# tskare/gpuaudiobench

Hardware: AMD Instinct MI355X
Metric: audio_buffers_per_sec (higher is better)
Workload: dtype f32

## Files before the change

gpuaudiobench_amd/csrc/k_conv_accel.hip:

```cpp
#include <hip/hip_runtime.h>
#include <hip/hip_ext.h>

#include <cmath>
#include <cstdlib>
#include <algorithm>
#include <chrono>
#include <memory>
#include <mutex>
#include <string>
#include <thread>
#include <type_traits>
#include <utility>
#include <vector>

#include "gab_common.hpp"
#include "gab_fft.hpp"
#include "gab_plan.hpp"
#include "k_conv_fdl.hpp"

namespace gab {
namespace fft {

void build_twiddles(float* t) {
    for (int m = 0; m < kTwiddleN; ++m) {
// ... 385 lines not shown
__global__ __launch_bounds__(kThreads) void conv_split_carry_refresh_kernel(
    const float* __restrict__ hist, const float4* __restrict__ pmF, cf* __restrict__ carry,
    const cf* __restrict__ tw, int head) {
    __shared__ cf lds[2 * kLdsHalf];
    const int tid = threadIdx.x;
    const int q = blockIdx.x;
    const cf* const hp = reinterpret_cast<const cf*>(hist) + (size_t)q * kSlots * kB;
    cf* const cp = carry + (size_t)q * kCarrySlots * kB;
    using FB = fft::BlockFFT<kNB, 16, false>;
    using FBi = fft::BlockFFT<kNB, 16, true>;
    cf* const X = lds;
    cf* const Y = lds + kLdsHalf;
    cf zb[16];
    typename FB::Bases twb_base;
    FB::load_twiddles(twb_base, tw, tid);
#pragma unroll
    for (int r = 0; r < 16; ++r)
        zb[r] = hp[((head + 1 + (r >> 1)) & (kSlots - 1)) * kB + (r & 1) * kThreads + tid];
    float4 cb[16];
    load_spectra<kNB, 16>(cb, pmF + (size_t)q * kBinsB, tid);
    typename FB::Twiddles twb;
    FB::expand_twiddles(twb_base, twb);
    FB::run(zb, X, Y, twb, tid);
    cf zpb[16];
    partner_exchange<kNB, 16, true>(zb, zpb, X, tid);
    spectral_product<kNB, 16>(zb, zpb, cb, tid);
    FBi::template run<typename FB::Twiddles, 4>(zb, Y, X, twb, tid);
    cf* const c1 = cp + ((head + 1) & (kCarrySlots - 1)) * kB;
    cf* const c2 = cp + ((head + 2) & (kCarrySlots - 1)) * kB;
    c1[tid] = zb[12];
    c1[tid + kThreads] = zb[13];
    c2[tid] = zb[14];
    c2[tid + kThreads] = zb[15];
}

constexpr unsigned kRtSentinel = 0xffa5c3e1u;
__device__ __forceinline__ bool rt_pending(unsigned w) { return (w >> 24) == (kRtSentinel >> 24); }
constexpr size_t kRtUploadPiece = (size_t(4) << 20) - 256;
constexpr int kRtPollLimit = 1 << 21;
constexpr int kRtMaxGroups = 40;
constexpr size_t kBatchChunk = 256;
struct ConvRoundTrip {
    unsigned* stage;
    float* park;
    float* h_out;
    unsigned* counters;
    unsigned* done;
    const unsigned* landed;
    unsigned* error;
    unsigned epoch;
    int groups;
    unsigned bound[kRtMaxGroups + 1];
};

#ifdef GAB_ABLATE
__device__ unsigned long long g_rt_stamps[65 * 4];
#define GAB_RT_STAMP_MIN(g, i) do { if (threadIdx.x == 0) atomicMin(&g_rt_stamps[(g) * 4 + (i)], (unsigned long long)__builtin_amdgcn_s_memrealtime()); } while (0)
#define GAB_RT_STAMP_MAX(g, i) do { if (threadIdx.x == 0) atomicMax(&g_rt_stamps[(g) * 4 + (i)], (unsigned long long)__builtin_amdgcn_s_memrealtime()); } while (0)
#else
#define GAB_RT_STAMP_MIN(g, i) do {} while (0)
#define GAB_RT_STAMP_MAX(g, i) do {} while (0)
#endif

__device__ __forceinline__ unsigned rt_peek(const unsigned* p) {
    return __hip_atomic_load(p, __ATOMIC_RELAXED, __HIP_MEMORY_SCOPE_SYSTEM);
}
constexpr unsigned kRtErrWait = 1u, kRtErrTorn = 2u;

__global__ __launch_bounds__(kThreads) void conv_round_trip_check_kernel(unsigned* __restrict__ stage, const float* __restrict__ hist,
                                                                        unsigned* __restrict__ verdict, int slot) {
    const int tid = threadIdx.x, q = blockIdx.x;
    const cf* const hp = reinterpret_cast<const cf*>(hist) + ((size_t)q * kSlots + slot) * kB;
    unsigned* const row = stage + (size_t)(2 * q) * kB;
    const cf c0 = hp[tid], c1 = hp[tid + kThreads];
    const unsigned v0 = rt_peek(row + tid), v1 = rt_peek(row + tid + kThreads), v2 = rt_peek(row + kB + tid), v3 = rt_peek(row + kB + tid + kThreads);
    const bool torn = v0 != __float_as_uint(c0.x) || v2 != __float_as_uint(c0.y) || v1 != __float_as_uint(c1.x) || v3 != __float_as_uint(c1.y);
    if (torn) __hip_atomic_fetch_or(verdict, kRtErrTorn, __ATOMIC_RELAXED, __HIP_MEMORY_SCOPE_SYSTEM);
    __hip_atomic_store(row + tid, kRtSentinel, __ATOMIC_RELAXED, __HIP_MEMORY_SCOPE_SYSTEM);
    __hip_atomic_store(row + tid + kThreads, kRtSentinel, __ATOMIC_RELAXED, __HIP_MEMORY_SCOPE_SYSTEM);
    __hip_atomic_store(row + kB + tid, kRtSentinel, __ATOMIC_RELAXED, __HIP_MEMORY_SCOPE_SYSTEM);
    __hip_atomic_store(row + kB + tid + kThreads, kRtSentinel, __ATOMIC_RELAXED, __HIP_MEMORY_SCOPE_SYSTEM);
}

__global__ __launch_bounds__(kThreads, 2) void conv_round_trip_kernel(
    ConvRoundTrip rt, float* __restrict__ hist, const float4* __restrict__ pmA, const float4* __restrict__ pmB,
    const cf* __restrict__ tw, int T, int head) {
    __shared__ cf lds[2 * kLdsHalf];
    __shared__ int s_word;
    cf* const lds0 = lds;
    cf* const lds1 = lds + kLdsHalf;
    const int tid = threadIdx.x;
    const int q = blockIdx.x;
    const int ta = 2 * q;
    int g = 0;
    while (q >= (int)rt.bound[g + 1]) ++g;
    GAB_RT_STAMP_MIN(g, 0);
    cf* const hp = reinterpret_cast<cf*>(hist) + (size_t)q * kSlots * kB;
    using FA = fft::BlockFFT<kNA, 4, false>;
    using FAi = fft::BlockFFT<kNA, 4, true>;
    using FB = fft::BlockFFT<kNB, 16, false>;
    using FBi = fft::BlockFFT<kNB, 16, true>;

    cf zb[16];
    typename FB::Bases twb_base;
    FB::load_twiddles(twb_base, tw, tid);
#pragma unroll
    for (int r = 0; r < 16; ++r) zb[r] = hp[((head + (r >> 1)) & (kSlots - 1)) * kB + (r & 1) * kThreads + tid];
    const cf prev0 = zb[14], prev1 = zb[15];
    {
        float4 cb[16];
        load_spectra<kNB, 16>(cb, pmB + (size_t)q * kBinsB, tid);
        __builtin_amdgcn_sched_barrier(0);
        typename FB::Twiddles twb;
        FB::expand_twiddles(twb_base, twb);
        FB::run(zb, lds1, lds0, twb, tid);
        cf zpb[16];
        partner_exchange<kNB, 16, true>(zb, zpb, lds1, tid);
        spectral_product<kNB, 16>(zb, zpb, cb, tid);
        FBi::template run<typename FB::Twiddles, 2>(zb, lds0, lds1, twb, tid);
    }
    const cf far0 = zb[14], far1 = zb[15];

    float4 ca[4];
    load_spectra<kNA, 4>(ca, pmA + (size_t)q * kBinsA, tid);
    typename FA::Twiddles twa;
    {
        typename FA::Bases twa_base;
        FA::load_twiddles(twa_base, tw, tid);
        FA::expand_twiddles(twa_base, twa);
    }

    const unsigned* const row = rt.stage + (size_t)ta * kB;
    if (tid == 0) {
        int tries = 0, bad = 0;
        while (rt_pending(rt_peek(row + 2 * kB - 1))) {
            if ((++tries & 63) == 0 && rt_peek(rt.landed) == rt.epoch) break;
            if (tries > kRtPollLimit) { bad = 1; break; }
            __builtin_amdgcn_s_sleep(30);
        }
        s_word = bad;
    }
    __syncthreads();
    bool gave_up = s_word != 0;
    unsigned w[4];
    {
        int tries = 0;
        for (;;) {
            w[0] = rt_peek(row + tid);
            w[1] = rt_peek(row + tid + kThreads);
            w[2] = rt_peek(row + kB + tid);
            w[3] = rt_peek(row + kB + tid + kThreads);
            if (gave_up || !(rt_pending(w[0]) || rt_pending(w[1]) || rt_pending(w[2]) || rt_pending(w[3]))) break;
            if ((++tries & 15) == 0 && __hip_atomic_load(rt.landed, __ATOMIC_ACQUIRE, __HIP_MEMORY_SCOPE_SYSTEM) == rt.epoch) {
                w[0] = rt_peek(row + tid);
                w[1] = rt_peek(row + tid + kThreads);
                w[2] = rt_peek(row + kB + tid);
                w[3] = rt_peek(row + kB + tid + kThreads);
                break;
            }
            if (tries > kRtPollLimit) { gave_up = true; break; }
            __builtin_amdgcn_s_sleep(10);
        }
    }
    GAB_RT_STAMP_MAX(g, 1);
    if (gave_up) __hip_atomic_store(rt.error, kRtErrWait, __ATOMIC_RELAXED, __HIP_MEMORY_SCOPE_SYSTEM);

    cf za[4];
    za[0] = prev0;
    za[1] = prev1;
    za[2] = mk(__uint_as_float(w[0]), __uint_as_float(w[2]));
    za[3] = mk(__uint_as_float(w[1]), __uint_as_float(w[3]));
    hp[head * kB + tid] = za[2];
    hp[head * kB + kThreads + tid] = za[3];
    __syncthreads();
    FA::run(za, lds0, lds1, twa, tid);
    {
        cf zpa[4];
        partner_exchange<kNA, 4, true>(za, zpa, lds0, tid);
        spectral_product<kNA, 4>(za, zpa, ca, tid);
    }
    FAi::run(za, lds1, lds0, twa, tid);
    float ya0 = 0.f, yb0 = 0.f, ya1 = 0.f, yb1 = 0.f;
    ya0 += za[2].x; yb0 += za[2].y; ya1 += za[3].x; yb1 += za[3].y;
    ya0 += far0.x; yb0 += far0.y; ya1 += far1.x; yb1 += far1.y;

    {
        unsigned long long* const p0 = reinterpret_cast<unsigned long long*>(rt.park + (size_t)T * tid + ta);
        unsigned long long* const p1 = reinterpret_cast<unsigned long long*>(rt.park + (size_t)T * (tid + kThreads) + ta);
        const unsigned long long v0 = ((unsigned long long)__float_as_uint(yb0) << 32) | __float_as_uint(ya0);
        const unsigned long long v1 = ((unsigned long long)__float_as_uint(yb1) << 32) | __float_as_uint(ya1);
        __hip_atomic_store(p0, v0, __ATOMIC_RELAXED, __HIP_MEMORY_SCOPE_AGENT);
        __hip_atomic_store(p1, v1, __ATOMIC_RELAXED, __HIP_MEMORY_SCOPE_AGENT);
    }
    asm volatile("s_waitcnt vmcnt(0)" ::: "memory");
    __syncthreads();
    GAB_RT_STAMP_MAX(g, 2);
    const int first = rt.bound[g];
    const int members = (int)rt.bound[g + 1] - first;
    unsigned* const gw = rt.counters + 32 * g;
    if (tid == 0) {
        const unsigned old = __hip_atomic_fetch_add(&gw[0], 1u, __ATOMIC_RELAXED, __HIP_MEMORY_SCOPE_AGENT);
        int role = 1;
        if (old + 1u == rt.epoch * (unsigned)members) {
            role = 2;
            __hip_atomic_store(&gw[1], 0u, __ATOMIC_RELAXED, __HIP_MEMORY_SCOPE_AGENT);
            asm volatile("s_waitcnt vmcnt(0)" ::: "memory");
            __hip_atomic_store(&gw[2], rt.epoch, __ATOMIC_RELAXED, __HIP_MEMORY_SCOPE_AGENT);
        } else {
            int tries = 0;
            while (__hip_atomic_load(&gw[2], __ATOMIC_RELAXED, __HIP_MEMORY_SCOPE_AGENT) != rt.epoch) {
                if (++tries > (1 << 10)) { role = 0; break; }
                __builtin_amdgcn_s_sleep(3);
            }
        }
        s_word = role;
    }
    __syncthreads();
    const int role = s_word;
    if (role == 0) return;
    const int row_f4 = members / 2;
    const auto srd = __builtin_amdgcn_make_buffer_rsrc(rt.park, 0, (int)((size_t)T * kB * 4), 0x00020000);
    const int col0 = 2 * first;
    unsigned drained = 0;
    for (;;) {
        __syncthreads();
        if (tid == 0) s_word = (int)__hip_atomic_fetch_add(&gw[1], 1u, __ATOMIC_RELAXED, __HIP_MEMORY_SCOPE_AGENT);
        __syncthreads();
        const int share = s_word;
        if (share >= members) break;
        const int i = share * kThreads + tid;
        const int sidx = i / row_f4, c = i - sidx * row_f4;
        const auto raw = __builtin_amdgcn_raw_buffer_load_b128(srd, 4u * (unsigned)(T * sidx + col0 + 4 * c), 0, 16);
        typedef float f4v __attribute__((ext_vector_type(4)));
        const f4v val = {__uint_as_float(raw[0]), __uint_as_float(raw[1]), __uint_as_float(raw[2]), __uint_as_float(raw[3])};
        float* const dst = rt.h_out + (size_t)T * sidx + col0 + 4 * c;
        asm volatile("global_store_dwordx4 %0, %1, off sc0 sc1" ::"v"(dst), "v"(val) : "memory");
        ++drained;
        if (role != 2) break;
    }
    asm volatile("s_waitcnt vmcnt(0)" ::: "memory");
    __syncthreads();
    GAB_RT_STAMP_MAX(g, 3);
    if (tid == 0 && drained) {
        const unsigned old = __hip_atomic_fetch_add(&rt.counters[32 * rt.groups], drained, __ATOMIC_RELAXED, __HIP_MEMORY_SCOPE_AGENT);
        if (old + drained == rt.epoch * (unsigned)gridDim.x) {
            __hip_atomic_store(rt.done, rt.epoch, __ATOMIC_RELAXED, __HIP_MEMORY_SCOPE_SYSTEM);
            GAB_RT_STAMP_MAX(64, 0);
        }
    }
}

__global__ __launch_bounds__(kThreads, 2) void conv_batch_kernel(
    const float* __restrict__ in, float* __restrict__ out, float* __restrict__ hist,
    const float4* __restrict__ pmA, const float4* __restrict__ pmB,
    const cf* __restrict__ tw, int T, int head, int n_buffers) {
    __shared__ cf lds[2 * kLdsHalf];
    const size_t step = (size_t)T * kB;
    for (int nb = 0; nb < n_buffers; ++nb)
        conv_one_buffer<true, true, true>(in + nb * step, out + nb * step, hist, pmA, pmB, tw, T,
                                             (head + nb) & (kSlots - 1), lds);
}

constexpr int kBatchBarriers = 6;

struct ConvEngine {
    const unsigned* doorbell;
    unsigned* relay;
    unsigned* progress;
    unsigned* completed;
    unsigned* error;
    int ring;
    int poll_every_period;
    unsigned* started;
    unsigned* resident;
    unsigned long long idle_ticks;
};
constexpr double kEngineIdleSeconds = 4.0;

typedef unsigned u4 __attribute__((ext_vector_type(4)));

constexpr int kB12Threads = 768;
constexpr int kB12SpecCf = 4 * kBinsA * 2;
constexpr int kB12Tw1Cf = 16 * 15;
constexpr int kB12Lds = 6 * kWaveImg + 2 * kLdsHalf + kB12SpecCf + kB12Tw1Cf;

template <int N, int R, int R0, int R1, class PM>
__device__ __forceinline__ void load_spectra_part(float4 (&c)[R1 - R0], PM pm, int tid) {
    constexpr int NT = N / R;
#pragma unroll
    for (int r = R0; r < R1; ++r) {
        const int k = tid + r * NT;
        if (r < R / 2) c[r - R0] = pm[k];
        else if (r > R / 2) c[r - R0] = pm[N - k];
        else c[r - R0] = pm[tid == 0 ? k : N - k];
    }
}
template <int N, int R, int R0, int R1>
__device__ __forceinline__ void spectral_product_part(cf (&z)[R], const cf (&zraw)[R1 - R0], const float4 (&c)[R1 - R0], int tid) {
#pragma unroll
    for (int r = R0; r < R1; ++r) {
        cf P = mk(c[r - R0].x, c[r - R0].y), M = mk(c[r - R0].z, c[r - R0].w);
        if (r > R / 2 || (r == R / 2 && tid != 0)) z[r] = fft::cfma_cjcj(zraw[r - R0], M, fft::cmulc(z[r], P));
        else z[r] = fft::cfma_cj(zraw[r - R0], M, fft::cmul(z[r], P));
    }
}
template <int R0, int R1>
__device__ __forceinline__ void near_product_half(cf (&v)[16], const cf* fimg, const float4* sp_lds, int lane) {
    cf zp[R1 - R0];
    float4 ch[R1 - R0];
#pragma unroll
    for (int r = R0; r < R1; ++r) zp[r - R0] = fimg[PadA16::at((kNA - (lane + 64 * r)) & (kNA - 1))];
    load_spectra_part<kNA, 16, R0, R1>(ch, sp_lds, lane);
    spectral_product_part<kNA, 16, R0, R1>(v, zp, ch, lane);
}

#ifdef GAB_ABLATE
__device__ unsigned long long g_split_stamps[2 * 8 * 8192];
#define GAB_B12BAR(period, i)                                                                                         \
    do {                                                                                                              \
        if ((sp.debug & 64) && ((period) == 32 || (period) == 33) && lane == 0)                                       \
            g_split_stamps[(((size_t)blockIdx.x * 12 + w) * 2 + ((period) - 32)) * 6 + (i)] = __builtin_amdgcn_s_memrealtime(); \
        __syncthreads();                                                                                              \
    } while (0)
#else
#define GAB_B12BAR(period, i) __syncthreads()
#endif
__device__ __forceinline__ void conv_split_batch12_resident(
    const float* __restrict__ in, float* __restrict__ out, float* __restrict__ hist,
    const float4* __restrict__ pmA, const ConvSplit& sp, const cf* __restrict__ tw, int T, int head0, int n_buffers,
    cf* __restrict__ lds) {
    cf* const far_img = lds + 6 * kWaveImg;
    float4* const spec = reinterpret_cast<float4*>(far_img + 2 * kLdsHalf);
    cf* const tw1 = reinterpret_cast<cf*>(spec + 4 * kBinsA);
    const int tid = threadIdx.x;
    const int d = xcd_contiguous(blockIdx.x, gridDim.x);
    const size_t step = (size_t)T * kB;
    {
        const float4* const gA = pmA + (size_t)(2 * d) * kBinsA;
        const float4* const gA2 = sp.pmA2 + (size_t)(2 * d) * kBinsA;
        for (int i = tid; i < 2 * kBinsA; i += kB12Threads) { spec[i] = gA[i]; spec[2 * kBinsA + i] = gA2[i]; }
        if (tid < 16) {
            cf pw[15];
            fft::powers_of<16>(tw[tid * (fft::kTwiddleN / 256)], pw);
#pragma unroll
            for (int r = 0; r < 15; ++r) tw1[tid * 15 + r] = pw[r];
        }
    }
    __syncthreads();
    const int lane = tid & 63;
    const int w = __builtin_amdgcn_readfirstlane(tid >> 6);
    const unsigned rb = (unsigned)lane + ((unsigned)lane >> 4);
    auto in_slot = [&](int slot) -> const float* { return in + (size_t)slot * step; };
    auto idle_period = [&]() { for (int i = 0; i < kBatchBarriers; ++i) __syncthreads(); };

    if (w >= 4) {
        const int g = __builtin_amdgcn_readfirstlane((w - 4) >> 2);
        const int ft = (tid - kThreads) & (kThreads - 1);
        cf* const img = far_img + g * kLdsHalf;
        const int q = 2 * d + g;
        const cf* const hp = reinterpret_cast<const cf*>(hist) + (size_t)q * kSlots * kB;
        cf* const cg = sp.carry + (size_t)q * kCarrySlots * kB;
        const size_t ca = (size_t)(2 * q) * kB, cb_ = ca + kB;
        const float4* const pf = sp.pmF + (size_t)q * kBinsB;
        using B16 = fft::Butterfly<16, false>;
        using B16i = fft::Butterfly<16, true>;
        cf tw2[15];
        fft::powers_of<16>(tw[ft], tw2);
        auto opaque_t = [&]() -> unsigned { unsigned v = (unsigned)ft; asm volatile("" : "+v"(v)); return v; };
        auto w0_of = [](unsigned t) -> unsigned { return t * 17u; };
        auto rd_of = [](unsigned t) -> unsigned { return t + (t >> 4); };
        auto w1_of = [](unsigned t) -> unsigned { const unsigned b1 = (t >> 4) * 256u + (t & 15u); return b1 + (b1 >> 4); };
        auto tw1row_of = [&](unsigned t) -> const cf* { return tw1 + (t & 15u) * 15u; };
        auto load_window = [&](auto part_tag, int nb, cf (&z)[16]) {
            constexpr int PART = decltype(part_tag)::value;
            const int head = (head0 + nb) & (kSlots - 1);
            int fo = ft;
            asm volatile("" : "+v"(fo));
            if constexpr (PART == 0) {
                const float* const cur = in_slot(nb);
                z[14] = mk(cur[ca + fo], cur[cb_ + fo]);
                z[15] = mk(cur[ca + fo + kThreads], cur[cb_ + fo + kThreads]);
            }
            constexpr int BL0 = PART == 0 ? 4 : 0, BL1 = PART == 0 ? 7 : 4;
            if (nb >= kSlots - 1) {
#pragma unroll
                for (int bl = BL0; bl < BL1; ++bl) {
                    const float* const src = in_slot(nb - (7 - bl));
                    z[2 * bl] = mk(src[ca + fo], src[cb_ + fo]);
                    z[2 * bl + 1] = mk(src[ca + fo + kThreads], src[cb_ + fo + kThreads]);
                }
            } else {
#pragma unroll
                for (int bl = BL0; bl < BL1; ++bl) {
                    if (nb - 7 + bl >= 0) {
                        const float* const src = in_slot(nb - (7 - bl));
                        z[2 * bl] = mk(src[ca + fo], src[cb_ + fo]);
                        z[2 * bl + 1] = mk(src[ca + fo + kThreads], src[cb_ + fo + kThreads]);
                    } else {
                        const int s = ((head + 1 + bl) & (kSlots - 1)) * kB;
                        z[2 * bl] = hp[s + fo];
                        z[2 * bl + 1] = hp[s + kThreads + fo];
                    }
                }
            }
        };
        cf z[16], zn[16];
        auto first_half = [&](int nb) {
#pragma unroll
            for (int r = 0; r < 16; ++r) z[r] = zn[r];
            B16::run(z);
            {
                const unsigned w0 = w0_of(opaque_t());
#pragma unroll
                for (int r = 0; r < 16; ++r) img[w0 + r] = z[B16::out_slot(r)];
            }
            GAB_B12BAR(nb, 0);
            {
                const unsigned t = opaque_t(), rd = rd_of(t);
                const cf* const tw1row = tw1row_of(t);
#pragma unroll
                for (int r = 0; r < 16; ++r) z[r] = img[rd + 272 * r];
#pragma unroll
                for (int r = 1; r < 16; ++r) z[r] = fft::cmul(z[r], tw1row[r - 1]);
            }
            B16::run(z);
            GAB_B12BAR(nb, 1);
            {
                const unsigned w1 = w1_of(opaque_t());
#pragma unroll
                for (int r = 0; r < 16; ++r) img[w1 + 17 * r] = z[B16::out_slot(r)];
            }
            __builtin_amdgcn_sched_barrier(0);
            float4 clo[8], chi[8];
            {
                int fo = ft;
                asm volatile("" : "+v"(fo));
                load_spectra_part<kNB, 16, 0, 8>(clo, pf, fo);
            }
            __builtin_amdgcn_sched_barrier(0);
            GAB_B12BAR(nb, 2);
            {
                const unsigned rd = rd_of(opaque_t());
#pragma unroll
                for (int r = 0; r < 16; ++r) z[r] = img[rd + 272 * r];
            }
#pragma unroll
            for (int r = 1; r < 16; ++r) z[r] = fft::cmul(z[r], tw2[r - 1]);
            __builtin_amdgcn_sched_barrier(0);
            {
                int fo = ft;
                asm volatile("" : "+v"(fo));
                load_spectra_part<kNB, 16, 8, 16>(chi, pf, fo);
            }
            __builtin_amdgcn_sched_barrier(0);
            B16::run(z);
            GAB_B12BAR(nb, 3);
            {
                const unsigned t = opaque_t();
#pragma unroll
                for (int r = 0; r < 16; ++r) img[t + 256u * r] = z[B16::out_slot(r)];
            }
            GAB_B12BAR(nb, 4);
            {
                cf o[16];
#pragma unroll
                for (int r = 0; r < 16; ++r) o[r] = z[B16::out_slot(r)];
#pragma unroll
                for (int r = 0; r < 16; ++r) z[r] = o[r];
                const unsigned t = opaque_t();
                const cf* const pb = img + (kNB - 256 * 15) - t;
                cf zp[8];
                zp[0] = img[(kNB - t) & (kNB - 1)];
#pragma unroll
                for (int r = 1; r < 8; ++r) zp[r] = pb[256 * (15 - r)];
                spectral_product_part<kNB, 16, 0, 8>(z, zp, clo, ft);
#pragma unroll
                for (int r = 0; r < 8; ++r) zp[r] = pb[256 * (7 - r)];
                spectral_product_part<kNB, 16, 8, 16>(z, zp, chi, ft);
            }
            B16i::run(z);
            GAB_B12BAR(nb, 5);
        };
        auto second_half = [&](int period, int nb_done, int nb_next) {
            if (nb_next >= 0) {
                load_window(std::integral_constant<int, 0>{}, nb_next, zn);
            } else {
#pragma unroll
                for (int r = 0; r < 16; ++r) zn[r] = mk(0.0f, 0.0f);
            }
            GAB_B12BAR(period, 0);
            if (nb_done >= 0) {
                const unsigned w0 = w0_of(opaque_t());
#pragma unroll
                for (int r = 0; r < 16; ++r) img[w0 + r] = z[B16i::out_slot(r)];
            }
            GAB_B12BAR(period, 1);
            if (nb_done >= 0) {
                const unsigned t = opaque_t(), rd = rd_of(t);
                const cf* const tw1row = tw1row_of(t);
#pragma unroll
                for (int r = 0; r < 16; ++r) z[r] = img[rd + 272 * r];
#pragma unroll
                for (int r = 1; r < 16; ++r) z[r] = fft::cmulc(z[r], tw1row[r - 1]);
                B16i::run(z);
            }
            GAB_B12BAR(period, 2);
            if (nb_done >= 0) {
                const unsigned w1 = w1_of(opaque_t());
#pragma unroll
                for (int r = 0; r < 16; ++r) img[w1 + 17 * r] = z[B16i::out_slot(r)];
            }
            __builtin_amdgcn_sched_barrier(0);
            if (nb_next >= 0) load_window(std::integral_constant<int, 1>{}, nb_next, zn);
            __builtin_amdgcn_sched_barrier(0);
            GAB_B12BAR(period, 3);
            if (nb_done >= 0) {
                const unsigned rd = rd_of(opaque_t());
#pragma unroll
                for (int r = 0; r < 16; ++r) z[r] = img[rd + 272 * r];
#pragma unroll
                for (int r = 1; r < 16; ++r) z[r] = fft::cmulc(z[r], tw2[r - 1]);
                cf x12, x13, x14, x15;
                B16i::run_last4(z, x12, x13, x14, x15);
                const int head = (head0 + nb_done) & (kSlots - 1);
                cf* const c1 = cg + ((head + 1) & (kCarrySlots - 1)) * kB;
                cf* const c2 = cg + ((head + 2) & (kCarrySlots - 1)) * kB;
                c1[ft] = x12;
                c1[ft + kThreads] = x13;
                c2[ft] = x14;
                c2[ft + kThreads] = x15;
            }
            GAB_B12BAR(period, 4);
            if (nb_done >= 0) asm volatile("s_waitcnt vmcnt(0)" ::: "memory");
            GAB_B12BAR(period, 5);
        };
        const int first = (g - head0) & 1;
        int nb = 0;
        if (first == 0 && n_buffers > 0) {
            load_window(std::integral_constant<int, 0>{}, 0, zn);
            load_window(std::integral_constant<int, 1>{}, 0, zn);
        }
        __syncthreads();
        if (first == 1) {
            second_half(0, -1, 1 < n_buffers ? 1 : -1);
            nb = 1;
        }
        for (;;) {
            if (nb > n_buffers) break;
            if (nb < n_buffers) first_half(nb); else idle_period();
            ++nb;
            if (nb > n_buffers) break;
            second_half(nb, nb - 1 < n_buffers ? nb - 1 : -1, nb + 1 < n_buffers ? nb + 1 : -1);
            ++nb;
        }
    } else if (w < 2) {
        const int q = 2 * d + w;
        cf* const hp = reinterpret_cast<cf*>(hist) + (size_t)q * kSlots * kB;
        cf* const img = lds + w * kWaveImg;
        cf* const hand = lds + (2 + w) * kWaveImg;
        const float4* const sa = spec + w * kBinsA;
        const float4* const sa2 = spec + (2 + w) * kBinsA;
        using WF = fft::WaveFFT1024<false>;
        WF::Lean t;
        WF::load_twiddles(t, tw, lane);
        const size_t xoff = (size_t)(2 * q) * kB;
        cf z[16], prev[8], nxt[8];
        {
            const int s1 = ((head0 + kSlots - 1) & (kSlots - 1)) * kB, s2 = ((head0 + kSlots - 2) & (kSlots - 1)) * kB;
#pragma unroll
            for (int j = 0; j < 8; ++j) z[j] = hp[s2 + lane + 64 * j];
#pragma unroll
            for (int j = 0; j < 8; ++j) prev[j] = hp[s1 + lane + 64 * j];
            if (n_buffers > 0) {
                const float* const x0 = in_slot(0) + xoff;
#pragma unroll
                for (int j = 0; j < 8; ++j) nxt[j] = mk(x0[lane + 64 * j], x0[kB + lane + 64 * j]);
            }
#pragma unroll
            for (int j = 0; j < 8; ++j) z[8 + j] = prev[j];
            WF::run(z, img, t, lane, WF::NoHook());
#pragma unroll
            for (int r = 0; r < 16; ++r) img[rb + 68 * r] = z[r];
            __syncthreads();
        }
        for (int nb = 0; nb < n_buffers; ++nb) {
            const int head = (head0 + nb) & (kSlots - 1);
            cf share[16];
#pragma unroll
            for (int r = 0; r < 8; ++r) share[r] = img[rb + 68 * r];
            near_product_half<0, 8>(share, img, sa2, lane);
            GAB_B12BAR(nb, 0);
            __builtin_amdgcn_sched_barrier(0);
#pragma unroll
            for (int j = 0; j < 8; ++j) { z[j] = prev[j]; z[8 + j] = nxt[j]; }
            if (nb + kSlots >= n_buffers) {
#pragma unroll
                for (int j = 0; j < 8; ++j) hp[head * kB + lane + 64 * j] = nxt[j];
            }
#pragma unroll
            for (int j = 0; j < 8; ++j) prev[j] = nxt[j];
            if (nb + 1 < n_buffers) {
                int lo = lane;
                asm volatile("" : "+v"(lo));
                const float* const xa = in_slot(nb + 1) + xoff + lo;
#pragma unroll
                for (int j = 0; j < 8; ++j) nxt[j] = mk(xa[64 * j], xa[kB + 64 * j]);
            }
            WF::run(z, img, t, lane, [&](int i) { GAB_B12BAR(nb, 1 + i); });
#pragma unroll
            for (int r = 0; r < 16; ++r) img[rb + 68 * r] = z[r];
            GAB_B12BAR(nb, 3);
            near_product_half<0, 8>(z, img, sa, lane);
            GAB_B12BAR(nb, 4);
#pragma unroll
            for (int r = 0; r < 8; ++r) hand[rb + 68 * r] = fft::cadd(z[r], share[r]);
            GAB_B12BAR(nb, 5);
        }
        idle_period();
    } else {
        const int pr = w - 2;
        cf* const hand = lds + (2 + pr) * kWaveImg;
        const cf* const fimg = lds + pr * kWaveImg;
        const float4* const sa = spec + pr * kBinsA;
        const float4* const sa2 = spec + (2 + pr) * kBinsA;
        cf* const img = lds + (4 + pr) * kWaveImg;
        const cf* const other = lds + (4 + (1 - pr)) * kWaveImg;
        const cf* const cg = sp.carry + (size_t)(2 * d + pr) * kCarrySlots * kB;
        using WFi = fft::WaveFFT1024<true>;
        WFi::Lean t;
        WFi::load_twiddles(t, tw, lane);
        cf ws[16], sum[8];
        auto product_half = [&](const float4* sp_lds) {
#pragma unroll
            for (int r = 8; r < 16; ++r) ws[r] = fimg[rb + 68 * r];
            near_product_half<8, 16>(ws, fimg, sp_lds, lane);
        };
        auto store_share = [&]() {
#pragma unroll
            for (int r = 8; r < 16; ++r) hand[rb + 68 * r] = ws[r];
        };
        auto sum_halves = [&]() {
#pragma unroll
            for (int j = 0; j < 8; ++j) sum[j] = fft::cadd(ws[8 + j], hand[rb + 68 * (8 + j)]);
        };
        __syncthreads();
        if (n_buffers > 0) {
            product_half(sa2);
            GAB_B12BAR(0, 0);
            store_share();
            GAB_B12BAR(0, 1);
            GAB_B12BAR(0, 2);
            GAB_B12BAR(0, 3);
            product_half(sa);
            GAB_B12BAR(0, 4);
            sum_halves();
            GAB_B12BAR(0, 5);
        } else {
            idle_period();
        }
        for (int nb = 1; nb <= n_buffers; ++nb) {
            const bool products = nb < n_buffers;
            const int b = nb - 1;
            const int head = (head0 + b) & (kSlots - 1);
            float* const outb = out + (size_t)b * step;
            cf z[16], y[8], park[8];
#pragma unroll
            for (int r = 0; r < 8; ++r) z[r] = hand[rb + 68 * r];
#pragma unroll
            for (int j = 0; j < 8; ++j) z[8 + j] = sum[j];
            {
                int lo = lane;
                asm volatile("" : "+v"(lo));
                const unsigned long long* const cy = reinterpret_cast<const unsigned long long*>(cg + (head & (kCarrySlots - 1)) * kB + lo);
#pragma unroll
                for (int j = 0; j < 8; ++j) {
                    const unsigned long long v = __hip_atomic_load(cy + 64 * j, __ATOMIC_RELAXED, __HIP_MEMORY_SCOPE_AGENT);
                    park[j] = mk(__uint_as_float((unsigned)v), __uint_as_float((unsigned)(v >> 32)));
                }
            }
            __builtin_amdgcn_sched_barrier(0);
            if (products) product_half(sa2);
            GAB_B12BAR(nb, 0);
            if (products) store_share();
            __builtin_amdgcn_sched_barrier(0);
            WFi::run(z, img, t, lane, [&](int i) { GAB_B12BAR(nb, 1 + i); });
#pragma unroll
            for (int j = 0; j < 8; ++j) y[j] = fft::cadd(z[8 + j], park[j]);
            GAB_B12BAR(nb, 3);
            if (pr == 0) {
#pragma unroll
                for (int j = 0; j < 4; ++j) img[lane + 64 * j] = y[4 + j];
            } else {
#pragma unroll
                for (int j = 0; j < 4; ++j) img[lane + 64 * j] = y[j];
            }
            __builtin_amdgcn_sched_barrier(0);
            if (products) product_half(sa);
            GAB_B12BAR(nb, 4);
            {
                float* const o0 = outb + 4 * (size_t)d;
                if (pr == 0) {
#pragma unroll
                    for (int j = 0; j < 4; ++j) {
                        const cf theirs = other[lane + 64 * j];
                        *reinterpret_cast<float4*>(o0 + (size_t)T * (lane + 64 * j)) = make_float4(y[j].x, y[j].y, theirs.x, theirs.y);
                    }
                } else {
#pragma unroll
                    for (int j = 0; j < 4; ++j) {
                        const cf theirs = other[lane + 64 * j];
                        *reinterpret_cast<float4*>(o0 + (size_t)T * (lane + 64 * (4 + j))) = make_float4(theirs.x, theirs.y, y[4 + j].x, y[4 + j].y);
                    }
                }
            }
            if (products) sum_halves();
            GAB_B12BAR(nb, 5);
        }
    }
}

__global__ __launch_bounds__(kB12Threads) void conv_split_batch12_kernel(
    const float* __restrict__ in, float* __restrict__ out, float* __restrict__ hist,
    const float4* __restrict__ pmA, ConvSplit sp, const cf* __restrict__ tw, int T, int head0, int n_buffers) {
    __shared__ __attribute__((aligned(16))) cf lds[kB12Lds];
    conv_split_batch12_resident(in, out, hist, pmA, sp, tw, T, head0, n_buffers, lds);
}

#ifdef GAB_ABLATE
#define GAB_E12BAR(i)                                                                                                 \
    do {                                                                                                              \
        if ((sp.debug & 64) && (nb == 4000 || nb == 4001) && lane == 0)                                               \
            g_split_stamps[(((size_t)blockIdx.x * 12 + w) * 2 + (nb - 4000)) * 6 + (i)] = __builtin_amdgcn_s_memrealtime(); \
        __syncthreads();                                                                                              \
    } while (0)
#else
#define GAB_E12BAR(i) __syncthreads()
#endif
__device__ __forceinline__ void conv_split_engine12_resident(
    const float* __restrict__ in, float* __restrict__ out, float* __restrict__ hist,
    const float4* __restrict__ pmA, const ConvSplit& sp, const cf* __restrict__ tw, int T, int head0,
    const ConvEngine& eng, cf* __restrict__ lds, unsigned* __restrict__ s_door) {
    constexpr bool ENGINE = true;
    constexpr int n_buffers = 0;
    (void)ENGINE; (void)n_buffers;
    cf* const far_img = lds + 6 * kWaveImg;
    float4* const spec = reinterpret_cast<float4*>(far_img + 2 * kLdsHalf);
    cf* const tw1 = reinterpret_cast<cf*>(spec + 4 * kBinsA);
    const int tid = threadIdx.x;
    const int d = xcd_contiguous(blockIdx.x, gridDim.x);
    const size_t step = (size_t)T * kB;
    {
        const float4* const gA = pmA + (size_t)(2 * d) * kBinsA;
        const float4* const gA2 = sp.pmA2 + (size_t)(2 * d) * kBinsA;
        for (int i = tid; i < 2 * kBinsA; i += kB12Threads) { spec[i] = gA[i]; spec[2 * kBinsA + i] = gA2[i]; }
        if (tid < 16) {
            cf pw[15];
            fft::powers_of<16>(tw[tid * (fft::kTwiddleN / 256)], pw);
#pragma unroll
            for (int r = 0; r < 15; ++r) tw1[tid * 15 + r] = pw[r];
        }
    }
    constexpr int kPoller = 2 * 64;
    auto read_door = [&]() -> unsigned {
        if (blockIdx.x == 0) {
            const unsigned v = __hip_atomic_load(eng.doorbell, __ATOMIC_RELAXED, __HIP_MEMORY_SCOPE_SYSTEM);
            __hip_atomic_store(eng.relay, v, __ATOMIC_RELAXED, __HIP_MEMORY_SCOPE_AGENT);
            return v;
        }
        return __hip_atomic_load(eng.relay, __ATOMIC_RELAXED, __HIP_MEMORY_SCOPE_AGENT);
    };
    if (tid == 0) {
        s_door[2] = 0;
        const unsigned before = __hip_atomic_fetch_add(eng.started, 1u, __ATOMIC_RELAXED, __HIP_MEMORY_SCOPE_AGENT);
        if (before == 0) __hip_atomic_store(&eng.resident[0], 1u, __ATOMIC_RELAXED, __HIP_MEMORY_SCOPE_SYSTEM);
        if (before + 1 == gridDim.x) __hip_atomic_store(&eng.resident[1], gridDim.x, __ATOMIC_RELAXED, __HIP_MEMORY_SCOPE_SYSTEM);
    }
    __syncthreads();
    const int lane = tid & 63;
    const int w = __builtin_amdgcn_readfirstlane(tid >> 6);
    const unsigned rb = (unsigned)lane + ((unsigned)lane >> 4);
    const bool aggregator = blockIdx.x == (gridDim.x > 1 ? 1u : 0u);
    unsigned reported = 0;
    auto aggregate_request = [&](u4& a, u4& b) {
        const auto srd = __builtin_amdgcn_make_buffer_rsrc(eng.progress, 0, (int)(8u * gridDim.x), 0x00020000);
        a = __builtin_amdgcn_raw_buffer_load_b128(srd, 32u * (unsigned)lane, 0, 16);
        b = __builtin_amdgcn_raw_buffer_load_b128(srd, 32u * (unsigned)lane + 16u, 0, 16);
    };
    auto aggregate_report = [&](const u4& a, const u4& b) {
        const unsigned words = 2u * gridDim.x;
        auto pick = [&](unsigned v, unsigned idx) { return idx < words ? v : 0xffffffffu; };
        unsigned m = min(min(min(pick(a[0], 8u * lane), pick(a[1], 8u * lane + 1)), min(pick(a[2], 8u * lane + 2), pick(a[3], 8u * lane + 3))),
// ... 1824 lines not shown
```

Measured before the change: 210,900.

## Compute spectral product via conjugate-pair partners to halve spectra loads

Instead of each thread loading spectra for all 16 bins and exchanging all bins through LDS, each thread now handles its low 8 bins and computes the products for their conjugate-symmetric partners itself. It writes those partner results to the upper half of the LDS image for the owning thread to read back before the inverse FFT, and the Nyquist bin is handled specially. This halves the global spectra loads and the LDS write volume, but adds an extra LDS round trip and moves the inverse butterfly into the second half of the pipeline. The old path is kept only behind an ablation debug flag.

```diff
diff --git a/gpuaudiobench_amd/csrc/k_conv_accel.hip b/gpuaudiobench_amd/csrc/k_conv_accel.hip
--- a/gpuaudiobench_amd/csrc/k_conv_accel.hip
+++ b/gpuaudiobench_amd/csrc/k_conv_accel.hip
@@ -711,6 +711,15 @@
         cf P = mk(c[r - R0].x, c[r - R0].y), M = mk(c[r - R0].z, c[r - R0].w);
         if (r > R / 2 || (r == R / 2 && tid != 0)) z[r] = fft::cfma_cjcj(zraw[r - R0], M, fft::cmulc(z[r], P));
         else z[r] = fft::cfma_cj(zraw[r - R0], M, fft::cmul(z[r], P));
+    }
+}
+template <int N, int R, int R0, int R1>
+__device__ __forceinline__ void spectral_product_partner_part(cf (&wp)[R1 - R0], const cf (&z)[R], const cf (&zp)[R1 - R0], const float4 (&c)[R1 - R0]) {
+    static_assert(R1 <= R / 2, "the partners of the low bins");
+#pragma unroll
+    for (int r = R0; r < R1; ++r) {
+        cf P = mk(c[r - R0].x, c[r - R0].y), M = mk(c[r - R0].z, c[r - R0].w);
+        wp[r - R0] = fft::cfma_cjcj(z[r], M, fft::cmulc(zp[r - R0], P));
     }
 }
 template <int R0, int R1>
@@ -814,6 +823,11 @@
             }
         };
         cf z[16], zn[16];
+#ifdef GAB_ABLATE
+        const bool own_bins = (sp.debug & 128) != 0;
+#else
+        constexpr bool own_bins = false;
+#endif
         auto first_half = [&](int nb) {
 #pragma unroll
             for (int r = 0; r < 16; ++r) z[r] = zn[r];
@@ -840,11 +854,12 @@
                 for (int r = 0; r < 16; ++r) img[w1 + 17 * r] = z[B16::out_slot(r)];
             }
             __builtin_amdgcn_sched_barrier(0);
-            float4 clo[8], chi[8];
+            float4 clo[8], cny = make_float4(0.0f, 0.0f, 0.0f, 0.0f);
             {
                 int fo = ft;
                 asm volatile("" : "+v"(fo));
                 load_spectra_part<kNB, 16, 0, 8>(clo, pf, fo);
+                if (fo == 0) cny = pf[kNB / 2];
             }
             __builtin_amdgcn_sched_barrier(0);
             GAB_B12BAR(nb, 2);
@@ -855,22 +870,16 @@
             }
 #pragma unroll
             for (int r = 1; r < 16; ++r) z[r] = fft::cmul(z[r], tw2[r - 1]);
-            __builtin_amdgcn_sched_barrier(0);
-            {
-                int fo = ft;
-                asm volatile("" : "+v"(fo));
-                load_spectra_part<kNB, 16, 8, 16>(chi, pf, fo);
-            }
-            __builtin_amdgcn_sched_barrier(0);
             B16::run(z);
             GAB_B12BAR(nb, 3);
-            {
-                const unsigned t = opaque_t();
-#pragma unroll
-                for (int r = 0; r < 16; ++r) img[t + 256u * r] = z[B16::out_slot(r)];
-            }
-            GAB_B12BAR(nb, 4);
-            {
+#ifdef GAB_ABLATE
+            if (own_bins) {
+                {
+                    const unsigned t = opaque_t();
+#pragma unroll
+                    for (int r = 0; r < 16; ++r) img[t + 256u * r] = z[B16::out_slot(r)];
+                }
+                GAB_B12BAR(nb, 4);
                 cf o[16];
 #pragma unroll
                 for (int r = 0; r < 16; ++r) o[r] = z[B16::out_slot(r)];
@@ -883,11 +892,44 @@
 #pragma unroll
                 for (int r = 1; r < 8; ++r) zp[r] = pb[256 * (15 - r)];
                 spectral_product_part<kNB, 16, 0, 8>(z, zp, clo, ft);
+                load_spectra_part<kNB, 16, 8, 16>(clo, pf, ft);
 #pragma unroll
                 for (int r = 0; r < 8; ++r) zp[r] = pb[256 * (7 - r)];
-                spectral_product_part<kNB, 16, 8, 16>(z, zp, chi, ft);
-            }
-            B16i::run(z);
+                spectral_product_part<kNB, 16, 8, 16>(z, zp, clo, ft);
+                GAB_B12BAR(nb, 5);
+                return;
+            }
+#endif
+            {
+                const unsigned t = opaque_t();
+#pragma unroll
+                for (int r = 8; r < 16; ++r) img[t + 256u * (r - 8)] = z[B16::out_slot(r)];
+            }
+            GAB_B12BAR(nb, 4);
+            {
+                cf o[16];
+#pragma unroll
+                for (int r = 0; r < 16; ++r) o[r] = z[B16::out_slot(r)];
+#pragma unroll
+                for (int r = 0; r < 16; ++r) z[r] = o[r];
+                const unsigned t = opaque_t();
+                const cf* const pb = img + (kNB / 2 - 256 * 7) - t;
+                cf zp[8], wp[8];
+                zp[0] = img[(kNB / 2 - t) & (kNB / 2 - 1)];
+                if (t == 0) zp[0] = z[0];
+#pragma unroll
+                for (int r = 1; r < 8; ++r) zp[r] = pb[256 * (7 - r)];
+                spectral_product_partner_part<kNB, 16, 0, 8>(wp, z, zp, clo);
+                spectral_product_part<kNB, 16, 0, 8>(z, zp, clo, ft);
+                if (t == 0) {
+                    const cf P = mk(cny.x, cny.y), M = mk(cny.z, cny.w);
+                    wp[0] = fft::cfma_cj(z[8], M, fft::cmul(z[8], P));
+                }
+                cf* const qb = img + kNB / 2 + (kNB / 2 - 256 * 7) - t;
+                img[kNB / 2 + ((kNB / 2 - t) & (kNB / 2 - 1))] = wp[0];
+#pragma unroll
+                for (int r = 1; r < 8; ++r) qb[256 * (7 - r)] = wp[r];
+            }
             GAB_B12BAR(nb, 5);
         };
         auto second_half = [&](int period, int nb_done, int nb_next) {
@@ -896,6 +938,15 @@
             } else {
 #pragma unroll
                 for (int r = 0; r < 16; ++r) zn[r] = mk(0.0f, 0.0f);
+            }
+            __builtin_amdgcn_sched_barrier(0);
+            if (nb_done >= 0) {
+                if (!own_bins) {
+                    const unsigned t = opaque_t();
+#pragma unroll
+                    for (int r = 8; r < 16; ++r) z[r] = img[kNB / 2 + t + 256u * (r - 8)];
+                }
+                B16i::run(z);
             }
             GAB_B12BAR(period, 0);
             if (nb_done >= 0) {
```

Result: faster. 215,200, median of 6 (+2.0%).
